# kyutai-labs/moshi

Hardware: AMD Instinct MI355X
Metric: 12.5 Hz frames/s end-to-end Mimi+Moshi-7B (higher is better)
Workload: dtype bf16

## Files before the change

### moshi_amd/csrc/mimi_engine.hip

```cpp
#include "mimi_kernels.h"
#include "mmi_graph.h"

#include <math.h>

namespace {

struct ConvW {
    float* wpk = nullptr;
    float* wpk_h = nullptr;
    float* bias = nullptr;
    int Cin = 0, Cout = 0, K = 1, S = 1, Mt = 0, Q = 0;
};

struct TrLayerW {
    ConvW in_proj, out_proj, lin1, lin2;
    float *n1w = nullptr, *n1b = nullptr, *n2w = nullptr, *n2b = nullptr, *ls1 = nullptr, *ls2 = nullptr;
    float *n1w_pk = nullptr, *n1b_pk = nullptr, *n2w_pk = nullptr, *n2b_pk = nullptr;
};

struct Buf {
    float* p = nullptr;
    int C = 0, ld = 0, H = 0;
    int lead = 0;
    float* pe = nullptr;
// ... 415 lines not shown
    }
    size_t n = (size_t)B * C * b->ld + b->lead;
    float* base = nullptr;
    MMI_HIP_CHECK(m->st.alloc(&base, n));
    MMI_HIP_CHECK(hipMemsetAsync(base, 0, n * sizeof(float), s));
    b->p = base + b->lead;
    return MMI_OK;
}

int alloc_twin(mmi_mimi* m, int B, Buf* b, hipStream_t s) {
    size_t n = (size_t)B * b->C * b->ld + b->lead;
    float* base = nullptr;
    MMI_HIP_CHECK(m->st.alloc(&base, n));
    MMI_HIP_CHECK(hipMemsetAsync(base, 0, n * sizeof(float), s));
    b->pe = base + b->lead;
    return MMI_OK;
}

HistDesc hist_of(const Buf& b, int T);
HistDesc hist_of_src(const Buf& b, int T) {
    Buf c = b;
    c.p = b.conv_src();
    return hist_of(c, T);
}

bool producer_packs(const mmi_mimi* m, int columns, const ConvW& w, int features) {
    return columns <= 128 && w.Q * 8 == features && !m->knobs.mimi_pack_launches;
}

int add_conv(mmi_mimi* m, MmiProgram& prog, ConvGemmArgs a, MmiArena* arena = nullptr) {
    ConvPlan p;
    int rc = plan_conv(m->knobs, arena ? *arena : m->st, a, &p);
    if (rc) return rc;
    prog.add([a, p](hipStream_t s) { return launch_conv_plan(s, a, p); });
    return MMI_OK;
}

int add_resblock(mmi_mimi* m, MmiProgram& prog, ConvGemmArgs a1, ConvGemmArgs a2, const ConvW& w2) {
    const int nblk = mmi_cdiv(a1.Ntot, 32);
    const long min_waves = m->knobs.res_fusion_min != MmiKnobs::UNSET ? m->knobs.res_fusion_min : 256;
    const bool fuse = a1.Ntot > 128 && a1.S == 1 && a2.K == 1 && a2.S == 1 && a1.Cout == a2.Cin && a1.Ntot == a2.Ntot &&
                      a1.T_out == a2.T_out && a1.Mt == 1 && w2.wpk_h && a2.Q <= 4 * a1.Mt &&
                      a2.Mt >= a1.Mt && (long)nblk * a1.Mt >= min_waves && !a1.first && !a2.first && !a1.res && !a1.scale && !a2.scale &&
                      a1.T_out % 32 == 0 && a1.Cin <= 64 * a1.Mt && a1.K <= 33 &&
                      a1.act_out == MMI_ACT_NONE && a2.act_out == MMI_ACT_NONE;
    if (!fuse) {
        int rc = add_conv(m, prog, a1);
        if (rc) return rc;
        return add_conv(m, prog, a2);
    }
    a2.wpk = w2.wpk_h;
    a2.elu_in = 0;
    ResBlockArgs ra;
    ra.a1 = a1; ra.a2 = a2;
    const int mt1 = a1.Mt;
    const size_t smem = ((size_t)((a1.Cin * (32 + a1.K - 1) + 3) & ~3) + (size_t)a1.Q * 8 + (mt1 > 1 ? (size_t)mt1 * 1024 : 0)) * sizeof(float);
    if (smem > 65536) return mmi_fail(MMI_ERR_UNSUPPORTED, "k_resblock: input window does not fit in LDS");
    prog.add([ra, nblk, smem](hipStream_t s) {
        MMI_LAUNCH((k_resblock<1, 4>), nblk, 64, smem, s, ra);
        MMI_CHECK_LAUNCH();
        return (int)MMI_OK;
    });
    return MMI_OK;
}

int add_quantize_ops(mmi_mimi* m, MmiProgram& prog, const float* latent, int lat_ld, int lat_off, int B, bool latent_packed = false) {
    const mmi_mimi_cfg& c = m->cfg;
    const int D = c.q_dimension, bins = c.q_bins;
    Buf in; in.p = const_cast<float*>(latent); in.C = c.dimension; in.ld = lat_ld; in.H = lat_off;
    Buf out; out.p = m->xq; out.C = 2 * D; out.ld = 1; out.H = 0;
    {
        ConvGemmArgs a = conv_args(m->q_in, in, lat_off, 1, out, 0, B, false);
        a.bp = m->qin_bp; a.partial = m->qin_part;
        a.x_packed = latent_packed ? 1 : 0;
        int rc = add_conv(m, prog, a);
        if (rc) return rc;
    }
    const int K = m->n_codebooks;
    const int nchunk = m->nchunk;
    const size_t smem = ((size_t)MMI_RVQ_CHUNK * (D + 4) + (size_t)8 * D) * sizeof(float);
    auto level = [&](int k, int slot) {
        const bool sem = k < c.q_n_q_semantic;
        RvqLevel L;
        L.x = m->xq + (sem ? 0 : D);
        L.E = m->E_all + (size_t)k * bins * D;
        L.e2 = m->e2_all + (size_t)k * bins;
        L.best_d = m->best_d + (size_t)slot * nchunk * m->max_batch;
        L.best_i = m->best_i + (size_t)slot * nchunk * m->max_batch;
        L.level = k;
        return L;
    };
    int* codes = m->codes_i32; const int nq = c.q_n_q;
    const bool pair = c.q_n_q_semantic == 1 && K >= 2 && !m->knobs.rvq_no_pair;
    for (int k = 0; k < K; ++k) {
        const RvqLevel a0 = level(k, 0);
        const bool two = pair && k == 0;
        const RvqLevel a1 = two ? level(1, 1) : a0;
        const int nz = two ? 2 : 1;
        prog.add([=](hipStream_t s) {
            MMI_LAUNCH(k_rvq_dist, dim3(nchunk, mmi_cdiv(B, 8), nz), 256, smem, s, a0, a1, 2 * D, B, D, bins);
            MMI_LAUNCH(k_rvq_select, dim3(B, nz), 256, 0, s, a0, a1, nchunk, 2 * D, codes, nq, B, D);
            MMI_CHECK_LAUNCH();
            return (int)MMI_OK;
        });
        if (two) ++k;
    }
    return MMI_OK;
}

int add_dequant_ops(mmi_mimi* m, MmiProgram& prog, int K, const Buf& out, int out_off, int B, bool k_from_device = false) {
    const mmi_mimi_cfg& c = m->cfg;
    const int D = c.q_dimension, bins = c.q_bins, nq = c.q_n_q, nsem = c.q_n_q_semantic;
    float* q2 = m->q2; const int* codes = m->dec_codes_i32; const float* E = m->E_all; const int* kdev = k_from_device ? m->dec_k_dev : nullptr;
    const bool packed = producer_packs(m, B, m->q_out, 2 * D);
    float* qp = packed ? m->qout_bp : nullptr; const int qQ = m->q_out.Q;
    prog.add([=](hipStream_t s) {
        MMI_LAUNCH(k_rvq_gather, mmi_cdiv(B * D, 256), 256, 0, s, codes, nq, K, E, bins, D, nsem, q2, B, kdev, qp, qQ);
        MMI_CHECK_LAUNCH();
        return (int)MMI_OK;
    });
    Buf in; in.p = m->q2; in.C = 2 * D; in.ld = 1; in.H = 0;
    ConvGemmArgs a = conv_args(m->q_out, in, 0, 1, out, out_off, B, false);
    a.bp = m->qout_bp; a.partial = m->qout_part;
    a.x_packed = packed ? 1 : 0;
    return add_conv(m, prog, a);
}

int add_transformer(mmi_mimi* m, MmiProgram& prog, const std::vector<TrLayerW>& layers, const Buf& xb, int off, int T,
                    float* kv, const long* offsets, int B, hipStream_t init_stream) {
    const mmi_mimi_cfg& c = m->cfg;
    const int d = c.tr_d_model, H = c.tr_num_heads, Dh = d / H, ff = c.tr_dim_feedforward, cap = c.tr_context;
    const int N = B * T;
    const bool packed = N <= 128;
    Buf y, qkv, att, hb;
    int rc;
    if ((rc = alloc_buf(m, B, d, 0, T, &y, init_stream))) return rc;
    if ((rc = alloc_buf(m, B, 3 * d, 0, T, &qkv, init_stream))) return rc;
    if ((rc = alloc_buf(m, B, d, 0, T, &att, init_stream))) return rc;
    if ((rc = alloc_buf(m, B, ff, 0, T, &hb, init_stream))) return rc;
    float *yp = nullptr, *attp = nullptr, *hbp = nullptr;
    const int nsub = mmi_cdiv(N, 32), Qd = mmi_cdiv(d, 8), Qff = mmi_cdiv(ff, 8);
    if (packed) {
        MMI_HIP_CHECK(m->st.alloc(&yp, (size_t)nsub * Qd * 256));
        MMI_HIP_CHECK(m->st.alloc(&attp, (size_t)nsub * Qd * 256));
        MMI_HIP_CHECK(m->st.alloc(&hbp, (size_t)nsub * Qff * 256));
        MMI_HIP_CHECK(hipMemsetAsync(yp, 0, (size_t)nsub * Qd * 256 * sizeof(float), init_stream));
        MMI_HIP_CHECK(hipMemsetAsync(attp, 0, (size_t)nsub * Qd * 256 * sizeof(float), init_stream));
        MMI_HIP_CHECK(hipMemsetAsync(hbp, 0, (size_t)nsub * Qff * 256 * sizeof(float), init_stream));
    }
    const size_t kv_layer = (size_t)B * H * cap * Dh;
    if (T > 2 || (Dh != 16 && Dh != 32 && Dh != 64))
        return mmi_fail(MMI_ERR_UNSUPPORTED, "Mimi attention: head dim 16/32/64 and 1 or 2 steps per frame are built");
    const size_t attn_smem = ((size_t)T * Dh + (((size_t)T * cap + 3) & ~(size_t)3) + (size_t)(256 / (Dh / 4)) * T * Dh + 8) * sizeof(float);
    auto add_norm = [&](const float* w, const float* bb) {
        const float* xp = xb.p; int xld = xb.ld; float* yn = y.p;
        prog.add([=](hipStream_t s) {
            MMI_LAUNCH(k_layernorm_ct, B * T, 64, 0, s, xp, xld, off, w, bb, yn, T, 0, d, T, 1e-5f, yp, Qd);
            MMI_CHECK_LAUNCH();
            return (int)MMI_OK;
        });
    };
    const bool fuse_ln = packed && d % 8 == 0 && Qd <= 64 && layers.size() > 0 && layers[0].n1w_pk;
    float* xrp = nullptr;
    if (fuse_ln) {
        MMI_HIP_CHECK(m->st.alloc(&xrp, (size_t)nsub * Qd * 256));
        MMI_HIP_CHECK(hipMemsetAsync(xrp, 0, (size_t)nsub * Qd * 256 * sizeof(float), init_stream));
    }
    bool x_is_packed = false;
    for (size_t l = 0; l < layers.size(); ++l) {
        const TrLayerW& L = layers[l];
        {
            ConvGemmArgs ai = conv_args(L.in_proj, y, 0, T, qkv, 0, B, false);
            if (fuse_ln && x_is_packed) {
                ai.x_packed = 1; ai.bp = xrp; ai.ln_w = L.n1w_pk; ai.ln_b = L.n1b_pk; ai.ln_eps = 1e-5f;
            } else {
                add_norm(L.n1w, L.n1b);
                if (packed) { ai.x_packed = 1; ai.bp = yp; }
            }
            if ((rc = add_conv(m, prog, ai))) return rc;
            MimiAttnArgs aa;
            aa.qkv = qkv.p; aa.kc = kv + (2 * l) * kv_layer; aa.vc = kv + (2 * l + 1) * kv_layer;
            aa.offsets = offsets; aa.out = att.p; aa.B = B; aa.H = H; aa.D = Dh; aa.T = T; aa.cap = cap;
            aa.context = c.tr_context; aa.max_period = c.tr_max_period;
            aa.outp = attp; aa.outQ = Qd;
            const bool one_pass = cap <= 16 * (256 / (Dh / 4)) && !m->knobs.mimi_attn_two_pass;
            prog.add([=](hipStream_t s) {
#define MMI_ATT(D_, T_) do { if (one_pass) MMI_LAUNCH((k_mimi_attn_1pass<D_, T_>), B * H, 256, 0, s, aa); \
                             else MMI_LAUNCH((k_mimi_attn<D_, T_>), B * H, 256, attn_smem, s, aa); } while (0)
                if (Dh == 64 && T == 2) MMI_ATT(64, 2);
                else if (Dh == 64 && T == 1) MMI_ATT(64, 1);
                else if (Dh == 32 && T == 2) MMI_ATT(32, 2);
                else if (Dh == 32 && T == 1) MMI_ATT(32, 1);
                else if (Dh == 16 && T == 2) MMI_ATT(16, 2);
                else if (Dh == 16 && T == 1) MMI_ATT(16, 1);
                else return mmi_fail(MMI_ERR_UNSUPPORTED, "Mimi attention: head dim 16/32/64 and 1 or 2 steps per frame are built");
#undef MMI_ATT
                MMI_CHECK_LAUNCH();
                return (int)MMI_OK;
            });
            ConvGemmArgs a = conv_args(L.out_proj, att, 0, T, xb, off, B, false);
            a.res = xb.p; a.res_ld = xb.ld; a.res_off = off; a.scale = L.ls1;
            if (packed) { a.x_packed = 1; a.bp = attp; }
            if (fuse_ln) { a.outp = xrp; a.outQ = Qd; x_is_packed = true; }
            if ((rc = add_conv(m, prog, a))) return rc;
        }
        {
            ConvGemmArgs a1 = conv_args(L.lin1, y, 0, T, hb, 0, B, false);
            a1.act_out = MMI_ACT_GELU;
            if (fuse_ln && x_is_packed) {
                a1.x_packed = 1; a1.bp = xrp; a1.ln_w = L.n2w_pk; a1.ln_b = L.n2b_pk; a1.ln_eps = 1e-5f;
                a1.out_mode = MMI_GOUT_PACKED; a1.outp = hbp; a1.outQ = Qff;
            } else {
                add_norm(L.n2w, L.n2b);
                if (packed) { a1.x_packed = 1; a1.bp = yp; a1.out_mode = MMI_GOUT_PACKED; a1.outp = hbp; a1.outQ = Qff; }
            }
            if ((rc = add_conv(m, prog, a1))) return rc;
            ConvGemmArgs a2 = conv_args(L.lin2, hb, 0, T, xb, off, B, false);
            a2.res = xb.p; a2.res_ld = xb.ld; a2.res_off = off; a2.scale = L.ls2;
            if (packed) { a2.x_packed = 1; a2.bp = hbp; }
            if (fuse_ln) { a2.outp = xrp; a2.outQ = Qd; x_is_packed = true; }
            if ((rc = add_conv(m, prog, a2))) return rc;
        }
    }
    return MMI_OK;
}

int upload_hist(mmi_mimi* m, std::vector<HistDesc>& h, int B, HistDesc** dev, int* n, int* rows, HistTable* tab = nullptr) {
    int acc = 0;
    std::vector<HistDesc> keep;
    for (auto& d : h) {
        if (d.H <= 0) continue;
        d.row_begin = acc;
        acc += B * d.C;
        keep.push_back(d);
    }
    *n = (int)keep.size();
    *rows = acc;
    if (tab) {
        memset(tab, 0, sizeof(*tab));
        tab->n = keep.size() <= MMI_HIST_MAX ? (int)keep.size() : -1;
        for (size_t i = 0; i < keep.size() && i < MMI_HIST_MAX; ++i) tab->d[i] = keep[i];
    }
    MMI_HIP_CHECK(m->st.alloc(dev, keep.size() ? keep.size() : 1));
    if (!keep.empty())
        MMI_HIP_CHECK(hipMemcpy(*dev, keep.data(), keep.size() * sizeof(HistDesc), hipMemcpyHostToDevice));
    return MMI_OK;
}

HistDesc hist_of(const Buf& b, int T) {
    HistDesc d;
    d.p = b.p; d.C = b.C; d.ld = b.ld; d.H = b.H; d.T = T; d.row_begin = 0;
    return d;
}

int add_commit(mmi_mimi* m, MmiProgram& prog, std::vector<HistDesc>& hist, int B, int T_tr, HistDesc** dev, int* n, int* n_rows, long* cnt,
               uint8_t* fi) {
    HistTable tab;
    int rc = upload_hist(m, hist, B, dev, n, n_rows, &tab);
    if (rc) return rc;
    HistDesc* hd = *dev; const int nh = *n, rows = *n_rows;
    const uint8_t* ex = m->exec;
    const bool one = tab.n >= 0 && !m->knobs.mimi_two_commits;
    prog.add([=](hipStream_t s) {
        if (one) {
            MMI_LAUNCH(k_commit_all, mmi_cdiv(rows + B, 256), 256, 0, s, tab, rows, ex, cnt, 1, T_tr, fi, B);
            MMI_CHECK_LAUNCH();
            return (int)MMI_OK;
        }
        if (rows > 0) MMI_LAUNCH(k_commit_history, mmi_cdiv(rows, 256), 256, 0, s, (const HistDesc*)hd, nh, rows, ex);
        MMI_LAUNCH(k_commit_counters, mmi_cdiv(B, 64), 64, 0, s, cnt, 1, T_tr, fi, ex, B);
        MMI_CHECK_LAUNCH();
        return (int)MMI_OK;
    });
    return MMI_OK;
}

int build_encoder(mmi_mimi* m, int B, hipStream_t s0) {
    const mmi_mimi_cfg& c = m->cfg;
    MmiProgram& prog = m->enc_prog;
    std::vector<HistDesc> hist;
    int rc;
    int T = c.frame_size;
    size_t ci = 0;
    if ((rc = alloc_buf(m, B, c.channels, c.kernel_size - 1, T, &m->enc_in, s0))) return rc;
    hist.push_back(hist_of(m->enc_in, T));
    Buf cur = m->enc_in;
    int mult = 1;
    {
        Buf nxt;
        if ((rc = alloc_buf(m, B, c.n_filters, c.residual_kernel_size - 1, T, &nxt, s0))) return rc;
        if ((rc = alloc_twin(m, B, &nxt, s0))) return rc;
        prog.site("enc.conv0");
        if ((rc = add_conv(m, prog, conv_args(m->enc_convs[ci++], cur, 0, T, nxt, nxt.H, B, false)))) return rc;
        hist.push_back(hist_of_src(nxt, T));
        cur = nxt;
    }
    for (int i = 0; i < c.n_ratios; ++i) {
        const int ratio = c.ratios[c.n_ratios - 1 - i];
        const int ch = mult * c.n_filters;
        Buf hid, nxt;
        if ((rc = alloc_buf(m, B, ch / c.compress, 0, T, &hid, s0))) return rc;
        if ((rc = alloc_buf(m, B, ch, ratio, T, &nxt, s0))) return rc;
        hid.elu = nxt.elu = true;
        prog.site("enc.res" + std::to_string(i));
        const ConvGemmArgs a1 = conv_args(m->enc_convs[ci++], cur, 0, T, hid, 0, B, true);
        const ConvW& w2 = m->enc_convs[ci++];
        ConvGemmArgs a = conv_args(w2, hid, 0, T, nxt, nxt.H, B, true);
        a.res = cur.p; a.res_ld = cur.ld; a.res_off = cur.H;
        if ((rc = add_resblock(m, prog, a1, a, w2))) return rc;
        hist.push_back(hist_of(nxt, T));
        cur = nxt;
        const int Tn = T / ratio;
        const int Hn = (i + 1 < c.n_ratios) ? c.residual_kernel_size - 1 : c.last_kernel_size - 1;
        Buf nx2;
        if ((rc = alloc_buf(m, B, 2 * ch, Hn, Tn, &nx2, s0))) return rc;
        if (i + 1 < c.n_ratios) { if ((rc = alloc_twin(m, B, &nx2, s0))) return rc; }
        else nx2.elu = true;
        prog.site("enc.down" + std::to_string(i));
        if ((rc = add_conv(m, prog, conv_args(m->enc_convs[ci++], cur, 0, Tn, nx2, nx2.H, B, true)))) return rc;
        hist.push_back(hist_of_src(nx2, Tn));
        cur = nx2;
        T = Tn;
        mult *= 2;
    }
    const int stride = c.resample_stride;
    Buf dsin;
    if ((rc = alloc_buf(m, B, c.dimension, 2 * stride - stride, T, &dsin, s0))) return rc;
    prog.site("enc.final");
    if ((rc = add_conv(m, prog, conv_args(m->enc_convs[ci++], cur, 0, T, dsin, dsin.H, B, true)))) return rc;
    hist.push_back(hist_of(dsin, T));
    {
        const int Dh = c.tr_d_model / c.tr_num_heads;
        size_t kvn = (size_t)2 * c.tr_num_layers * B * c.tr_num_heads * c.tr_context * Dh;
        MMI_HIP_CHECK(m->st.alloc(&m->enc_kv, kvn));
        MMI_HIP_CHECK(hipMemsetAsync(m->enc_kv, 0, kvn * sizeof(float), s0));
        prog.site("enc.tr");
        if ((rc = add_transformer(m, prog, m->enc_tr, dsin, dsin.H, T, m->enc_kv, m->counters, B, s0))) return rc;
    }
    const int T_tr = T;
    if (T % stride != 0 || T / stride != 1)
// ... 491 lines not shown
```

### moshi_amd/csrc/mimi_kernels.h

```cpp
#pragma once
#include "mmi_common.h"

__global__ void k_pack_a_f32(const float* __restrict__ W, float* __restrict__ P, int M, int Kd, long sm, long sk,
                             int Mt, int Q) {
    long idx = (long)blockIdx.x * blockDim.x + threadIdx.x;
    long total = (long)Mt * Q * 256;
    if (idx >= total) return;
    int e = (int)(idx & 3);
    int lane = (int)((idx >> 2) & 63);
    long rest = idx >> 8;
    int q = (int)(rest % Q);
    int mt = (int)(rest / Q);
    int m = mt * 32 + (lane & 31);
    int kd = (q * 4 + e) * 2 + (lane >> 5);
    float v = 0.f;
    if (m < M && kd < Kd) v = W[(long)m * sm + (long)kd * sk];
    P[idx] = v;
}

__global__ void k_copy2d_f32(const float* __restrict__ src, long sld, float* __restrict__ dst, long dld, int rows,
                             int cols) {
    long idx = (long)blockIdx.x * blockDim.x + threadIdx.x;
    if (idx >= (long)rows * cols) return;
    int r = (int)(idx / cols), c = (int)(idx % cols);
// ... 665 lines not shown
    float pv[8];
#pragma unroll
    for (int s = 0; s < 8; ++s) pv[s] = a.partial[((long)min(s, ksplit - 1) * a.Mt * 32 + co) * a.Npad + n];
    float x = 0.f;
#pragma unroll
    for (int s = 0; s < 8; ++s) x += s < ksplit ? pv[s] : 0.f;
    const int bq = mmi_fast_div(n, a.T_magic);
    int co1[1] = {co}, b1[1] = {bq}, t1[1] = {n - bq * a.T_out};
    bool ok1[1] = {true};
    float v1[1] = {x};
    mmi_conv_store_n<1>(a, co1, b1, t1, ok1, v1);
}

__global__ void k_convtr_combine(const float* __restrict__ tmp, const float* __restrict__ bias,
                                 float* __restrict__ partial, const uint8_t* __restrict__ exec, float* __restrict__ out,
                                 int out_ld, int out_off, int B, int Cout, int K, int S, int T_in, float* __restrict__ out2,
                                 int tmp_ld) {
    long idx = (long)blockIdx.x * blockDim.x + threadIdx.x;
    const int Tout = T_in * S;
    if (idx >= (long)B * Cout * Tout) return;
    int p = (int)(idx % Tout);
    long row = idx / Tout;
    int co = (int)(row % Cout);
    int b = (int)(row / Cout);
    int t = p / S, r = p - t * S;
    const float* trow = tmp + row * (long)K * tmp_ld;
    float v = trow[(long)r * tmp_ld + t];
    if (t > 0) v += trow[(long)(r + S) * tmp_ld + (t - 1)];
    if (bias) v += bias[co];
    if (t == 0) {
        long pi = row * (long)(K - S) + r;
        v += partial[pi];
        if (exec[b]) partial[pi] = trow[(long)(r + S) * tmp_ld + (T_in - 1)];
    }
    out[row * (long)out_ld + out_off + p] = v;
    if (out2) out2[row * (long)out_ld + out_off + p] = mmi_elu(v);
}

__global__ void k_upsample_dw(const float* __restrict__ x, int x_ld, int x_off, const float* __restrict__ w,
                              float* __restrict__ partial, const uint8_t* __restrict__ exec, float* __restrict__ out,
                              int out_ld, int out_off, int B, int C, int K, int S, int T_in) {
    long idx = (long)blockIdx.x * blockDim.x + threadIdx.x;
    const int Tout = T_in * S;
    if (idx >= (long)B * C * Tout) return;
    int p = (int)(idx % Tout);
    long row = idx / Tout;
    int c = (int)(row % C);
    int b = (int)(row / C);
    int t = p / S, r = p - t * S;
    const float* xr = x + row * (long)x_ld + x_off;
    float v = w[c * K + r] * xr[t];
    if (t > 0) v += w[c * K + r + S] * xr[t - 1];
    if (t == 0) {
        long pi = row * (long)(K - S) + r;
        v += partial[pi];
        if (exec[b]) partial[pi] = w[c * K + r + S] * xr[T_in - 1];
    }
    out[row * (long)out_ld + out_off + p] = v;
}

struct HistDesc {
    float* p;
    int C, ld, H, T;
    int row_begin;
};

__global__ void k_commit_history(const HistDesc* __restrict__ descs, int ndesc, int total_rows,
                                 const uint8_t* __restrict__ exec) {
    int gid = (int)(blockIdx.x * blockDim.x + threadIdx.x);
    if (gid >= total_rows) return;
    int d = 0;
    while (d + 1 < ndesc && descs[d + 1].row_begin <= gid) ++d;
    HistDesc h = descs[d];
    int row = gid - h.row_begin;
    int b = row / h.C;
    if (!exec[b]) return;
    float* r = h.p + (long)row * h.ld;
    for (int p = 0; p < h.H; ++p) r[p] = r[p + h.T];
}

#define MMI_HIST_MAX 16
struct HistTable {
    HistDesc d[MMI_HIST_MAX];
    int n;
};
__global__ void k_commit_all(HistTable tab, int total_rows, const uint8_t* __restrict__ exec, long* __restrict__ counters,
                             int n_counters, int inc, uint8_t* __restrict__ first, int B) {
    int gid = (int)(blockIdx.x * blockDim.x + threadIdx.x);
    if (gid >= total_rows) {
        gid -= total_rows;
        if (gid >= B || !exec[gid]) return;
        for (int i = 0; i < n_counters; ++i) counters[(long)i * B + gid] += inc;
        if (first) first[gid] = 0;
        return;
    }
    int d = 0;
#pragma unroll
    for (int i = 1; i < MMI_HIST_MAX; ++i)
        if (i < tab.n && tab.d[i].row_begin <= gid) d = i;
    const HistDesc h = tab.d[d];
    int row = gid - h.row_begin;
    int b = row / h.C;
    if (!exec[b]) return;
    float* r = h.p + (long)row * h.ld;
    for (int p = 0; p < h.H; ++p) r[p] = r[p + h.T];
}

__global__ void k_commit_counters(long* __restrict__ counters, int n_counters, int inc, uint8_t* __restrict__ first,
                                  const uint8_t* __restrict__ exec, int B) {
    int gid = (int)(blockIdx.x * blockDim.x + threadIdx.x);
    if (gid >= B) return;
    if (!exec[gid]) return;
    for (int i = 0; i < n_counters; ++i) counters[(long)i * B + gid] += inc;
    if (first) first[gid] = 0;
}

__global__ void k_reset_history(const HistDesc* __restrict__ descs, int ndesc, int total_rows,
                                const uint8_t* __restrict__ mask) {
    int gid = (int)(blockIdx.x * blockDim.x + threadIdx.x);
    if (gid >= total_rows) return;
    int d = 0;
    while (d + 1 < ndesc && descs[d + 1].row_begin <= gid) ++d;
    HistDesc h = descs[d];
    int row = gid - h.row_begin;
    int b = row / h.C;
    if (mask && !mask[b]) return;
    float* r = h.p + (long)row * h.ld;
    for (int p = 0; p < h.H; ++p) r[p] = 0.f;
}

__global__ void k_reset_rows_f32(float* __restrict__ buf, long n_per_row, int B, const uint8_t* __restrict__ mask) {
    long idx = (long)blockIdx.x * blockDim.x + threadIdx.x;
    if (idx >= (long)B * n_per_row) return;
    int b = (int)(idx / n_per_row);
    if (mask && !mask[b]) return;
    buf[idx] = 0.f;
}

__global__ void k_reset_counters(long* __restrict__ counters, int n_counters, uint8_t* __restrict__ first,
                                 uint8_t* __restrict__ exec, int B, const uint8_t* __restrict__ mask) {
    int gid = (int)(blockIdx.x * blockDim.x + threadIdx.x);
    if (gid >= B) return;
    if (mask && !mask[gid]) return;
    for (int i = 0; i < n_counters; ++i) counters[(long)i * B + gid] = 0;
    if (first) first[gid] = 1;
    exec[gid] = 1;
}

__global__ void k_set_mask(uint8_t* __restrict__ dst, const uint8_t* __restrict__ src, int B) {
    int gid = (int)(blockIdx.x * blockDim.x + threadIdx.x);
    if (gid < B) dst[gid] = src[gid] ? 1 : 0;
}

__global__ __launch_bounds__(64) void k_layernorm_ct(const float* __restrict__ x, int x_ld, int x_off,
                                                     const float* __restrict__ w, const float* __restrict__ bvec,
                                                     float* __restrict__ y, int y_ld, int y_off, int C, int T,
                                                     float eps, float* __restrict__ yp, int yQ) {
    const int b = blockIdx.x / T, t = blockIdx.x % T;
    const int lane = threadIdx.x;
    const float* xc = x + (long)b * C * x_ld + x_off + t;
    constexpr int NR = 16;
    float xv[NR], wv[NR], bv[NR];
    float s = 0.f;
#pragma unroll
    for (int i = 0; i < NR; ++i) {
        const int c = lane + i * 64;
        const int cc = c < C ? c : 0;
        xv[i] = xc[(long)cc * x_ld];
        wv[i] = w[cc];
        bv[i] = bvec[cc];
    }
#pragma unroll
    for (int i = 0; i < NR; ++i) s += (lane + i * 64) < C ? xv[i] : 0.f;
#pragma unroll
    for (int m = 32; m >= 1; m >>= 1) s += mmi_shfl_xor(s, m);
    const float mean = s / (float)C;
    float v = 0.f;
#pragma unroll
    for (int i = 0; i < NR; ++i) {
        const float d = xv[i] - mean;
        v += (lane + i * 64) < C ? d * d : 0.f;
    }
#pragma unroll
    for (int m = 32; m >= 1; m >>= 1) v += mmi_shfl_xor(v, m);
    const float rstd = mmi_rsqrtf(v / (float)C + eps);
    float* yc = y + (long)b * C * y_ld + y_off + t;
#pragma unroll
    for (int i = 0; i < NR; ++i) {
        const int c = lane + i * 64;
        if (c < C) {
            const float o = (xv[i] - mean) * rstd * wv[i] + bv[i];
            if (yp) yp[mmi_bp_index(c, blockIdx.x, yQ)] = o;
            else yc[(long)c * y_ld] = o;
        }
    }
}

struct MimiAttnArgs {
    const float* qkv;
    float* kc;
    float* vc;
    const long* offsets;
    float* out;
    float* outp;
    int outQ;
    int B, H, D, T, cap, context;
    float max_period;
};

template <int D, int T>
__global__ __launch_bounds__(256) void k_mimi_attn(MimiAttnArgs a) {
    constexpr int LPR = D / 4;
    constexpr int RPB = 256 / LPR;
    const int b = blockIdx.x / a.H, h = blockIdx.x % a.H;
    const int tid = threadIdx.x, lane = tid & 63, wave = tid >> 6;
    const int cap = a.cap;
    MMI_DYN_SHARED(float, sm);
    float* qs = sm;
    float* sc = qs + T * D;
    float* red = sc + ((T * cap + 3) & ~3);
    const long off = a.offsets[b];
    const int HD = a.H * D;
    const float* qrow = a.qkv + (long)b * 3 * HD * T;
    float* kcb = a.kc + ((long)b * a.H + h) * cap * D;
    float* vcb = a.vc + ((long)b * a.H + h) * cap * D;

    for (int i = tid; i < T * (D / 2); i += 256) {
        const int t = i / (D / 2), j = i % (D / 2);
        const float freq = expf((float)j * (-logf(a.max_period) * 2.0f / (float)D));
        const float ts = (float)(off + t);
        const float ang = freq * ts;
        const float c = cosf(ang), s = sinf(ang);
        const float qr = qrow[(long)(h * D + 2 * j) * T + t], qi = qrow[(long)(h * D + 2 * j + 1) * T + t];
        const float kr = qrow[(long)(HD + h * D + 2 * j) * T + t], ki = qrow[(long)(HD + h * D + 2 * j + 1) * T + t];
        float q_re, q_im, k_re, k_im;
        mmi_rope_rotate(qr, qi, c, s, q_re, q_im);
        mmi_rope_rotate(kr, ki, c, s, k_re, k_im);
        qs[t * D + 2 * j] = q_re;
        qs[t * D + 2 * j + 1] = q_im;
        const int slot = (int)((off + t) % cap);
        kcb[(long)slot * D + 2 * j] = k_re;
        kcb[(long)slot * D + 2 * j + 1] = k_im;
    }
    for (int i = tid; i < T * D; i += 256) {
        const int t = i / D, d = i % D;
        const int slot = (int)((off + t) % cap);
        vcb[(long)slot * D + d] = qrow[(long)(2 * HD + h * D + d) * T + t];
    }
    __syncthreads();

    const long last = off + T - 1;
    const int end_index = (int)(last % cap);
    const long end_new = off + T;
    const int L = (int)(end_new < (long)cap ? end_new : (long)cap);
    const float scale = 1.0f / sqrtf((float)D);
    const int seg = tid % LPR, rsub = tid / LPR;
    f32x4 qv[T];
#pragma unroll
    for (int t = 0; t < T; ++t) qv[t] = *reinterpret_cast<const f32x4*>(qs + t * D + seg * 4);
    constexpr int NP = 8;
    for (int s0 = 0; s0 < L; s0 += NP * RPB) {
        f32x4 kk[NP];
#pragma unroll
        for (int i = 0; i < NP; ++i) kk[i] = *reinterpret_cast<const f32x4*>(kcb + (long)min(s0 + i * RPB + rsub, L - 1) * D + seg * 4);
#pragma unroll
        for (int i = 0; i < NP; ++i) {
            const int slot = s0 + i * RPB + rsub;
            const int delta = slot - end_index;
            const long pos = delta <= 0 ? last + delta : last + delta - cap;
#pragma unroll
            for (int t = 0; t < T; ++t) {
                float dv = (qv[t][0] * kk[i][0] + qv[t][1] * kk[i][1]) + (qv[t][2] * kk[i][2] + qv[t][3] * kk[i][3]);
#pragma unroll
                for (int m = LPR / 2; m >= 1; m >>= 1) dv += mmi_shfl_xor(dv, m);
                if (seg == 0 && slot < L) {
                    const long dq = (off + t) - pos;
                    const bool ok = pos >= 0 && dq >= 0 && dq < a.context;
                    sc[t * cap + slot] = ok ? dv * scale : -INFINITY;
                }
            }
        }
    }
    __syncthreads();

    if (wave < T) {
        const int t = wave;
        float m = -INFINITY;
        for (int slot = lane; slot < L; slot += 64) m = fmaxf(m, sc[t * cap + slot]);
#pragma unroll
        for (int x = 32; x >= 1; x >>= 1) m = fmaxf(m, mmi_shfl_xor(m, x));
        float sum = 0.f;
        for (int slot = lane; slot < L; slot += 64) {
            const float e = expf(sc[t * cap + slot] - m);
            sc[t * cap + slot] = e;
            sum += e;
        }
#pragma unroll
        for (int x = 32; x >= 1; x >>= 1) sum += mmi_shfl_xor(sum, x);
        const float inv = 1.0f / sum;
        for (int slot = lane; slot < L; slot += 64) sc[t * cap + slot] *= inv;
    }
    __syncthreads();

    float acc[T][4];
#pragma unroll
    for (int t = 0; t < T; ++t)
#pragma unroll
        for (int e = 0; e < 4; ++e) acc[t][e] = 0.f;
    for (int s0 = 0; s0 < L; s0 += NP * RPB) {
        f32x4 vv[NP];
#pragma unroll
        for (int i = 0; i < NP; ++i) vv[i] = *reinterpret_cast<const f32x4*>(vcb + (long)min(s0 + i * RPB + rsub, L - 1) * D + seg * 4);
#pragma unroll
        for (int i = 0; i < NP; ++i) {
            const int slot = s0 + i * RPB + rsub;
#pragma unroll
            for (int t = 0; t < T; ++t) {
                const float pr = slot < L ? sc[t * cap + slot] : 0.f;
#pragma unroll
                for (int e = 0; e < 4; ++e) acc[t][e] += pr * vv[i][e];
            }
        }
    }
#pragma unroll
    for (int t = 0; t < T; ++t)
        *reinterpret_cast<f32x4*>(red + (rsub * T + t) * D + seg * 4) = f32x4{acc[t][0], acc[t][1], acc[t][2], acc[t][3]};
    __syncthreads();
    for (int i = tid; i < T * D; i += 256) {
        const int t = i / D, d = i % D;
        float s = 0.f;
#pragma unroll 8
        for (int r = 0; r < RPB; ++r) s += red[(r * T + t) * D + d];
        if (a.outp) a.outp[mmi_bp_index(h * D + d, b * T + t, a.outQ)] = s;
        else a.out[((long)b * HD + h * D + d) * T + t] = s;
    }
}

template <int D, int T>
__global__ __launch_bounds__(256) void k_mimi_attn_1pass(MimiAttnArgs a) {
    constexpr int LPR = D / 4;
    constexpr int RPB = 256 / LPR;
    constexpr int IT = 16;
    const int b = blockIdx.x / a.H, h = blockIdx.x % a.H;
    const int tid = threadIdx.x, lane = tid & 63, wave = tid >> 6;
    const int cap = a.cap;
    MMI_SHARED __attribute__((aligned(16))) float qs[T * D];
    MMI_SHARED __attribute__((aligned(16))) float kn[T * D];
    MMI_SHARED __attribute__((aligned(16))) float vn[T * D];
    MMI_SHARED __attribute__((aligned(16))) float red[4 * T * D];
    MMI_SHARED float mw[4 * T];
    MMI_SHARED float sw[4 * T];
    const long off = a.offsets[b];
    const int HD = a.H * D;
    const float* qrow = a.qkv + (long)b * 3 * HD * T;
    float* kcb = a.kc + ((long)b * a.H + h) * cap * D;
    float* vcb = a.vc + ((long)b * a.H + h) * cap * D;
    const long last = off + T - 1;
    const int end_index = (int)(last % cap);
    const long end_new = off + T;
    const int L = (int)(end_new < (long)cap ? end_new : (long)cap);
    const int seg = tid % LPR, rsub = tid / LPR;

    f32x4 kk[IT], vv[IT];
#pragma unroll
    for (int i = 0; i < IT; ++i) {
        const long r = (long)min(i * RPB + rsub, L - 1) * D + seg * 4;
        kk[i] = *reinterpret_cast<const f32x4*>(kcb + r);
        vv[i] = *reinterpret_cast<const f32x4*>(vcb + r);
    }

    for (int i = tid; i < T * (D / 2); i += 256) {
        const int t = i / (D / 2), j = i % (D / 2);
        const float freq = expf((float)j * (-logf(a.max_period) * 2.0f / (float)D));
        const float ang = freq * (float)(off + t);
        const float c = cosf(ang), s = sinf(ang);
        const float qr = qrow[(long)(h * D + 2 * j) * T + t], qi = qrow[(long)(h * D + 2 * j + 1) * T + t];
        const float kr = qrow[(long)(HD + h * D + 2 * j) * T + t], ki = qrow[(long)(HD + h * D + 2 * j + 1) * T + t];
        mmi_rope_rotate(qr, qi, c, s, qs[t * D + 2 * j], qs[t * D + 2 * j + 1]);
        mmi_rope_rotate(kr, ki, c, s, kn[t * D + 2 * j], kn[t * D + 2 * j + 1]);
    }
    for (int i = tid; i < T * D; i += 256) {
        const int t = i / D, d = i % D;
        vn[i] = qrow[(long)(2 * HD + h * D + d) * T + t];
    }
    __syncthreads();
    for (int i = tid; i < T * D; i += 256) {
        const int t = i / D, d = i % D;
        const long slot = (off + t) % cap;
        kcb[slot * D + d] = kn[i];
        vcb[slot * D + d] = vn[i];
    }

    const float scale = 1.0f / sqrtf((float)D);
    f32x4 qv[T];
    int newslot[T];
#pragma unroll
    for (int t = 0; t < T; ++t) {
        qv[t] = *reinterpret_cast<const f32x4*>(qs + t * D + seg * 4);
        newslot[t] = (int)((off + t) % cap);
    }
    float sc[T][IT];
    float mx[T];
#pragma unroll
    for (int t = 0; t < T; ++t) mx[t] = -INFINITY;
#pragma unroll
    for (int i = 0; i < IT; ++i) {
        const int slot = i * RPB + rsub;
#pragma unroll
        for (int t = 0; t < T; ++t)
            if (slot == newslot[t]) {
                kk[i] = *reinterpret_cast<const f32x4*>(kn + t * D + seg * 4);
                vv[i] = *reinterpret_cast<const f32x4*>(vn + t * D + seg * 4);
            }
        const int delta = slot - end_index;
        const long pos = delta <= 0 ? last + delta : last + delta - cap;
#pragma unroll
        for (int t = 0; t < T; ++t) {
            float dv = (qv[t][0] * kk[i][0] + qv[t][1] * kk[i][1]) + (qv[t][2] * kk[i][2] + qv[t][3] * kk[i][3]);
#pragma unroll
            for (int m = LPR / 2; m >= 1; m >>= 1) dv += mmi_shfl_xor(dv, m);
            const long dq = (off + t) - pos;
            const bool ok = slot < L && pos >= 0 && dq >= 0 && dq < a.context;
            sc[t][i] = ok ? dv * scale : -INFINITY;
            mx[t] = fmaxf(mx[t], sc[t][i]);
        }
    }
    float acc[T][4], sum[T];
#pragma unroll
    for (int t = 0; t < T; ++t) {
#pragma unroll
        for (int m = LPR; m < 64; m <<= 1) mx[t] = fmaxf(mx[t], mmi_shfl_xor(mx[t], m));
        const float mref = mx[t] == -INFINITY ? 0.f : mx[t];
        sum[t] = 0.f;
#pragma unroll
        for (int e = 0; e < 4; ++e) acc[t][e] = 0.f;
#pragma unroll
        for (int i = 0; i < IT; ++i) {
            const float p = expf(sc[t][i] - mref);
            sum[t] += p;
#pragma unroll
            for (int e = 0; e < 4; ++e) acc[t][e] += p * vv[i][e];
        }
#pragma unroll
        for (int m = LPR; m < 64; m <<= 1) {
            sum[t] += mmi_shfl_xor(sum[t], m);
#pragma unroll
            for (int e = 0; e < 4; ++e) acc[t][e] += mmi_shfl_xor(acc[t][e], m);
        }
        if (lane < LPR) {
            *reinterpret_cast<f32x4*>(red + (wave * T + t) * D + seg * 4) = f32x4{acc[t][0], acc[t][1], acc[t][2], acc[t][3]};
            if (lane == 0) { mw[wave * T + t] = mx[t]; sw[wave * T + t] = sum[t]; }
        }
    }
    __syncthreads();
    for (int i = tid; i < T * D; i += 256) {
        const int t = i / D, d = i % D;
        float m = mw[t];
#pragma unroll
        for (int w = 1; w < 4; ++w) m = fmaxf(m, mw[w * T + t]);
        float num = 0.f, den = 0.f;
#pragma unroll
        for (int w = 0; w < 4; ++w) {
            const float f = expf(mw[w * T + t] - m);
            num += f * red[(w * T + t) * D + d];
            den += f * sw[w * T + t];
        }
        const float o = num / den;
        if (a.outp) a.outp[mmi_bp_index(h * D + d, b * T + t, a.outQ)] = o;
        else a.out[((long)b * HD + h * D + d) * T + t] = o;
    }
}

#define MMI_RVQ_CHUNK 32
struct RvqLevel {
    float* x;
    const float* E;
    const double* e2;
    double* best_d;
    int* best_i;
    int level;
};

__global__ __launch_bounds__(256) void k_rvq_dist(RvqLevel l0, RvqLevel l1, int x_rstride, int Bn, int D, int bins) {
    const RvqLevel& L = blockIdx.z == 0 ? l0 : l1;
    const float* __restrict__ x = L.x;
    const float* __restrict__ E = L.E;
    const double* __restrict__ e2 = L.e2;
    double* __restrict__ best_d = L.best_d;
    int* __restrict__ best_i = L.best_i;
    MMI_DYN_SHARED(float, sm);
    const int ldE = D + 4;
    float* Es = sm;
    float* xs = sm + MMI_RVQ_CHUNK * ldE;
    const int chunk = blockIdx.x;
    const int c0 = chunk * MMI_RVQ_CHUNK;
    const int tid = threadIdx.x;
    const int rg0 = (int)blockIdx.y * 8;
    const int D4 = D >> 2;
    {
        const int r = tid >> 3, j0 = tid & 7;
        const int code = min(c0 + r, bins - 1);
        for (int j = j0; j < D4; j += 8)
            *reinterpret_cast<f32x4*>(Es + r * ldE + 4 * j) = *reinterpret_cast<const f32x4*>(E + (long)code * D + 4 * j);
        if (r < 8) {
            const int row = min(rg0 + r, Bn - 1);
            for (int j = j0; j < D4; j += 8)
                *reinterpret_cast<f32x4*>(xs + r * D + 4 * j) = *reinterpret_cast<const f32x4*>(x + (long)row * x_rstride + 4 * j);
        }
    }
    __syncthreads();
    const int c = tid & 31, g = tid >> 5;
    const bool cvalid = (c0 + c) < bins;
    const double en = cvalid ? e2[c0 + c] : 0.0;
    const int r = rg0 + g;
    const bool rvalid = r < Bn;
    double a0 = 0.0, a1 = 0.0, a2 = 0.0, a3 = 0.0;
    for (int j = 0; j < D4; ++j) {
        const f32x4 ev = *reinterpret_cast<const f32x4*>(Es + c * ldE + 4 * j);
        const f32x4 xv = *reinterpret_cast<const f32x4*>(xs + g * D + 4 * j);
        a0 += (double)ev[0] * (double)xv[0];
        a1 += (double)ev[1] * (double)xv[1];
        a2 += (double)ev[2] * (double)xv[2];
        a3 += (double)ev[3] * (double)xv[3];
    }
    const double acc = (a0 + a1) + (a2 + a3);
    double dist = (cvalid && rvalid) ? en - 2.0 * acc : INFINITY;
    int idx = c0 + c;
#pragma unroll
    for (int m = 16; m >= 1; m >>= 1) {
        double od = mmi_shfl_xor(dist, m);
        int oi = mmi_shfl_xor(idx, m);
        if (od < dist || (od == dist && oi < idx)) { dist = od; idx = oi; }
    }
    if (c == 0 && rvalid) { best_d[(long)chunk * Bn + r] = dist; best_i[(long)chunk * Bn + r] = idx; }
}

__global__ __launch_bounds__(256) void k_rvq_select(RvqLevel l0, RvqLevel l1, int nchunk, int x_rstride, int* __restrict__ codes,
                                                    int codes_rstride, int Bn, int D) {
    const RvqLevel& L = blockIdx.y == 0 ? l0 : l1;
    const double* __restrict__ best_d = L.best_d;
    const int* __restrict__ best_i = L.best_i;
    float* __restrict__ x = L.x;
    const float* __restrict__ E = L.E;
    const int level = L.level;
    const int r = blockIdx.x;
    MMI_SHARED int widx;
    if (threadIdx.x < 64) {
        double bd = INFINITY;
        int bi = 0x7fffffff;
        for (int ch = threadIdx.x; ch < nchunk; ch += 64) {
            double d = best_d[(long)ch * Bn + r];
            int i = best_i[(long)ch * Bn + r];
            if (d < bd || (d == bd && i < bi)) { bd = d; bi = i; }
        }
#pragma unroll
        for (int m = 32; m >= 1; m >>= 1) {
            double od = mmi_shfl_xor(bd, m);
            int oi = mmi_shfl_xor(bi, m);
            if (od < bd || (od == bd && oi < bi)) { bd = od; bi = oi; }
        }
// ... 47 lines not shown
```

### moshi_amd/csrc/mmi_knobs.h

```cpp
#pragma once
#include <limits.h>
#include <stdio.h>
#include <stdlib.h>
#include <atomic>
#include <string>
#include <vector>

struct MmiKnobs {
    static constexpr int UNSET = INT_MIN;

    bool no_graph = false;
    char debug_poison = 0;
    std::vector<std::string> skip_sites;

    int lm_tile = 0;
    int dep_tile = 0;
    bool no_dep_in_group = false;
    int gemm_ksplit = 0;
    bool gemm_osplit_set = false;
    int gemm_osplit = UNSET;
    bool gemm_osplit_all = false;
    char gemm_lds = 0;
    int gemm_lds_grid = UNSET;
    char gemm_once = 0;
    bool no_norm_fusion = false;
    bool q8_act_bf16 = false;
    bool q8_u2 = false;
    bool q8_tiles_serial = false;
    bool rows_groups = false;
    int rows_ntw = 0;
    bool attn_split = false;
    int attn_ns = 0;
    int attn_solo = UNSET;
    bool attn_merge_kernel = false;
    bool no_dep_attn_fusion = false;
    bool dep_attn0_launch = false;
    bool no_precapture = false;
    bool debug_trace = false;
    std::string debug_trace_prefix;
    std::string debug_dump;

    int conv_mtb = 0;
    int conv_w = 0;
    int conv_ksplit = 0;
    long res_fusion_min = UNSET;
    bool mimi_no_align = false;
    bool rvq_no_pair = false;
    bool mimi_pack_launches = false;
    bool mimi_attn_two_pass = false;
    bool mimi_two_commits = false;

    int duplex_codec_cus = 0;
    char duplex_prio = 0;
};

inline void mmi_knob_warn_once(std::atomic<bool>& said, const char* name, const char* value, const char* what) {
    if (!said.exchange(true)) fprintf(stderr, "moshi_mi: %s=%s is set: %s\n", name, value, what);
}

inline MmiKnobs mmi_knobs_from_env() {
    MmiKnobs k;
    auto present = [](const char* name) { return getenv(name) != nullptr; };
    auto first = [](const char* name) { const char* e = getenv(name); return e ? e[0] : (char)0; };
    auto number = [](const char* name, int absent) { const char* e = getenv(name); return e ? atoi(e) : absent; };
    auto one_of = [](int v, std::initializer_list<int> ok) { for (int o : ok) if (v == o) return v; return 0; };

    {
        const char* e = getenv("MMI_NO_GRAPH");
        k.no_graph = e && e[0] && e[0] != '0';
    }
    {
        const char p = first("MMI_DEBUG_POISON");
        k.debug_poison = p == '1' || p == '0' ? p : (char)0;
    }
    if (const char* e = getenv("MMI_SKIP_SITES")) {
        const std::string all(e);
        for (size_t i = 0; i <= all.size();) {
            const size_t j = all.find(',', i);
            const std::string pre = all.substr(i, j == std::string::npos ? std::string::npos : j - i);
            if (!pre.empty()) k.skip_sites.push_back(pre);
            if (j == std::string::npos) break;
            i = j + 1;
        }
        static std::atomic<bool> said{false};
        if (!k.skip_sites.empty()) mmi_knob_warn_once(said, "MMI_SKIP_SITES", e, "launch-list sites are left out, the outputs are garbage (timing experiments only)");
    }

    k.lm_tile = one_of(number("MMI_LM_TILE", 0), {16, 32});
    k.dep_tile = number("MMI_DEP_TILE", 0);
    k.no_dep_in_group = present("MMI_NO_DEP_IN_GROUP");
    {
        const int v = number("MMI_GEMM_KSPLIT", 0);
        k.gemm_ksplit = v >= 1 && v <= 4 ? v : 0;
    }
    if (const char* e = getenv("MMI_GEMM_OSPLIT")) {
        k.gemm_osplit_set = true;
        if (e[0]) { k.gemm_osplit = atoi(e); k.gemm_osplit_all = e[1] == 'a'; }
    }
    k.gemm_lds = first("MMI_GEMM_LDS");
    k.gemm_lds_grid = number("MMI_GEMM_LDS_GRID", MmiKnobs::UNSET);
    k.gemm_once = first("MMI_GEMM_ONCE");
    k.no_norm_fusion = present("MMI_NO_NORM_FUSION");
    k.q8_act_bf16 = first("MMI_Q8_ACT") == 'b';
    k.q8_u2 = first("MMI_Q8_U") == '2';
    k.q8_tiles_serial = first("MMI_Q8_TILES") == 's';
    {
        const char* e = getenv("MMI_ROWS_GROUPS");
        k.rows_groups = e && e[0] && e[0] != '0';
    }
    k.rows_ntw = one_of(number("MMI_ROWS_NTW", 0), {1, 2});
    k.attn_split = first("MMI_ATTN") == 's';
    {
        const int v = number("MMI_ATTN_NS", 0);
        k.attn_ns = v >= 1 && v <= 16 ? v : 0;
    }
    k.attn_solo = number("MMI_ATTN_SOLO", MmiKnobs::UNSET);
    k.attn_merge_kernel = first("MMI_ATTN_MERGE") == 'k';
    k.no_dep_attn_fusion = present("MMI_NO_DEP_ATTN_FUSION");
    k.dep_attn0_launch = present("MMI_DEP_ATTN0_LAUNCH");
    k.no_precapture = present("MMI_NO_PRECAPTURE");
    if (const char* e = getenv("MMI_DEBUG_TRACE")) { k.debug_trace = true; k.debug_trace_prefix = e; }
    if (const char* e = getenv("MMI_DEBUG_DUMP")) k.debug_dump = e;

    k.conv_mtb = one_of(number("MMI_CONV_MTB", 0), {1, 2, 4});
    k.conv_w = one_of(number("MMI_CONV_W", 0), {1, 2, 4, 8});
    {
        const int v = number("MMI_CONV_KSPLIT", 0);
        k.conv_ksplit = v >= 1 && v <= 8 ? v : 0;
    }
    if (const char* e = getenv("MMI_MIMI_RES_FUSION_MIN")) k.res_fusion_min = atol(e);
    k.mimi_no_align = present("MMI_MIMI_NO_ALIGN");
    k.rvq_no_pair = present("MMI_RVQ_NO_PAIR");
    k.mimi_pack_launches = present("MMI_MIMI_PACK_LAUNCHES");
    k.mimi_attn_two_pass = present("MMI_MIMI_ATTN_TWO_PASS");
    k.mimi_two_commits = present("MMI_MIMI_TWO_COMMITS");

    if (const char* e = getenv("MMI_DUPLEX_CODEC_CUS")) {
        const int v = atoi(e);
        static std::atomic<bool> said{false};
        if (v > 0 && v < 256) {
            k.duplex_codec_cus = v;
            mmi_knob_warn_once(said, "MMI_DUPLEX_CODEC_CUS", e, "the duplex pipeline's codec streams run on a CU mask (experiment)");
        } else if (e[0]) mmi_knob_warn_once(said, "MMI_DUPLEX_CODEC_CUS", e, "ignored, the CU count must be 1..255");
    }
    if (const char* e = getenv("MMI_DUPLEX_PRIO")) {
        static std::atomic<bool> said{false};
        if (e[0] == 'c' || e[0] == 'n') {
            k.duplex_prio = e[0];
            mmi_knob_warn_once(said, "MMI_DUPLEX_PRIO", e, "the duplex pipeline's stream priorities are not the shipped ones (A/B)");
        } else if (e[0]) mmi_knob_warn_once(said, "MMI_DUPLEX_PRIO", e, "ignored, the values are codec / none");
    }
    return k;
}
```

Baseline: 4480.

## Precompute Mimi RoPE table in layernorm launch and prefetch KV before offset load

Extra blocks are added to the first layernorm launch of each transformer so they compute the cos/sin RoPE table once per frame. The one-pass attention kernel then reads this table instead of evaluating expf/cosf/sinf in every layer and head. The kernel also issues its first K/V cache loads before reading the offset, clamping them to the cache capacity, and zeroes V for slots past the valid length. The aim is to cut transcendental work and hide load latency, at the cost of a small buffer and extra blocks in the layernorm launch.

```diff
diff --git a/moshi_amd/csrc/mimi_engine.hip b/moshi_amd/csrc/mimi_engine.hip
--- a/moshi_amd/csrc/mimi_engine.hip
+++ b/moshi_amd/csrc/mimi_engine.hip
@@ -591,10 +591,21 @@
     if (T > 2 || (Dh != 16 && Dh != 32 && Dh != 64))
         return mmi_fail(MMI_ERR_UNSUPPORTED, "Mimi attention: head dim 16/32/64 and 1 or 2 steps per frame are built");
     const size_t attn_smem = ((size_t)T * Dh + (((size_t)T * cap + 3) & ~(size_t)3) + (size_t)(256 / (Dh / 4)) * T * Dh + 8) * sizeof(float);
+    const bool one_pass = cap <= 16 * (256 / (Dh / 4)) && !m->knobs.mimi_attn_two_pass;
+    float* rope = nullptr;
+    if (one_pass && !m->knobs.mimi_rope_in_kernel && !layers.empty()) {
+        MMI_HIP_CHECK(m->st.alloc(&rope, (size_t)N * Dh));
+        MMI_HIP_CHECK(hipMemsetAsync(rope, 0, (size_t)N * Dh * sizeof(float), init_stream));
+    }
+    bool rope_filled = false;
+    const float max_period = c.tr_max_period;
     auto add_norm = [&](const float* w, const float* bb) {
         const float* xp = xb.p; int xld = xb.ld; float* yn = y.p;
+        float* rp = rope_filled ? nullptr : rope;
+        rope_filled = true;
         prog.add([=](hipStream_t s) {
-            MMI_LAUNCH(k_layernorm_ct, B * T, 64, 0, s, xp, xld, off, w, bb, yn, T, 0, d, T, 1e-5f, yp, Qd);
+            MMI_LAUNCH(k_layernorm_ct, rp ? 2 * B * T : B * T, 64, 0, s, xp, xld, off, w, bb, yn, T, 0, d, T, 1e-5f, yp, Qd, B * T, rp, offsets, Dh,
+                       max_period);
             MMI_CHECK_LAUNCH();
             return (int)MMI_OK;
         });
@@ -621,10 +632,10 @@
             aa.qkv = qkv.p; aa.kc = kv + (2 * l) * kv_layer; aa.vc = kv + (2 * l + 1) * kv_layer;
             aa.offsets = offsets; aa.out = att.p; aa.B = B; aa.H = H; aa.D = Dh; aa.T = T; aa.cap = cap;
             aa.context = c.tr_context; aa.max_period = c.tr_max_period;
-            aa.outp = attp; aa.outQ = Qd;
-            const bool one_pass = cap <= 16 * (256 / (Dh / 4)) && !m->knobs.mimi_attn_two_pass;
+            aa.outp = attp; aa.outQ = Qd; aa.rope = rope;
             prog.add([=](hipStream_t s) {
-#define MMI_ATT(D_, T_) do { if (one_pass) MMI_LAUNCH((k_mimi_attn_1pass<D_, T_>), B * H, 256, 0, s, aa); \
+#define MMI_ATT(D_, T_) do { if (one_pass && rope) MMI_LAUNCH((k_mimi_attn_1pass<D_, T_, true>), B * H, 256, 0, s, aa); \
+                             else if (one_pass) MMI_LAUNCH((k_mimi_attn_1pass<D_, T_, false>), B * H, 256, 0, s, aa); \
                              else MMI_LAUNCH((k_mimi_attn<D_, T_>), B * H, 256, attn_smem, s, aa); } while (0)
                 if (Dh == 64 && T == 2) MMI_ATT(64, 2);
                 else if (Dh == 64 && T == 1) MMI_ATT(64, 1);
diff --git a/moshi_amd/csrc/mimi_kernels.h b/moshi_amd/csrc/mimi_kernels.h
--- a/moshi_amd/csrc/mimi_kernels.h
+++ b/moshi_amd/csrc/mimi_kernels.h
@@ -841,12 +841,31 @@
     if (gid < B) dst[gid] = src[gid] ? 1 : 0;
 }
 
+__device__ __forceinline__ void mmi_mimi_rope_cs(float max_period, int D, long pos, int j, float& c, float& sn) {
+    const float freq = expf((float)j * (-logf(max_period) * 2.0f / (float)D));
+    const float ang = freq * (float)pos;
+    c = cosf(ang);
+    sn = sinf(ang);
+}
+
 __global__ __launch_bounds__(64) void k_layernorm_ct(const float* __restrict__ x, int x_ld, int x_off,
                                                      const float* __restrict__ w, const float* __restrict__ bvec,
                                                      float* __restrict__ y, int y_ld, int y_off, int C, int T,
-                                                     float eps, float* __restrict__ yp, int yQ) {
+                                                     float eps, float* __restrict__ yp, int yQ,
+                                                     int n_norm, float* __restrict__ rope, const long* __restrict__ offsets, int Dh,
+                                                     float max_period) {
+    const int lane = threadIdx.x;
+    if (blockIdx.x >= n_norm) {
+        const int bt = (int)blockIdx.x - n_norm;
+        const long pos = offsets[bt / T] + bt % T;
+        if (lane < Dh / 2) {
+            float c, sn;
+            mmi_mimi_rope_cs(max_period, Dh, pos, lane, c, sn);
+            *reinterpret_cast<f32x2*>(rope + ((long)bt * (Dh / 2) + lane) * 2) = f32x2{c, sn};
+        }
+        return;
+    }
     const int b = blockIdx.x / T, t = blockIdx.x % T;
-    const int lane = threadIdx.x;
     const float* xc = x + (long)b * C * x_ld + x_off + t;
     constexpr int NR = 16;
     float xv[NR], wv[NR], bv[NR];
@@ -895,6 +914,7 @@
     int outQ;
     int B, H, D, T, cap, context;
     float max_period;
+    const float* rope;
 };
 
 template <int D, int T>
@@ -916,10 +936,8 @@
 
     for (int i = tid; i < T * (D / 2); i += 256) {
         const int t = i / (D / 2), j = i % (D / 2);
-        const float freq = expf((float)j * (-logf(a.max_period) * 2.0f / (float)D));
-        const float ts = (float)(off + t);
-        const float ang = freq * ts;
-        const float c = cosf(ang), s = sinf(ang);
+        float c, s;
+        mmi_mimi_rope_cs(a.max_period, D, off + t, j, c, s);
         const float qr = qrow[(long)(h * D + 2 * j) * T + t], qi = qrow[(long)(h * D + 2 * j + 1) * T + t];
         const float kr = qrow[(long)(HD + h * D + 2 * j) * T + t], ki = qrow[(long)(HD + h * D + 2 * j + 1) * T + t];
         float q_re, q_im, k_re, k_im;
@@ -1025,11 +1043,12 @@
     }
 }
 
-template <int D, int T>
+template <int D, int T, bool TAB>
 __global__ __launch_bounds__(256) void k_mimi_attn_1pass(MimiAttnArgs a) {
     constexpr int LPR = D / 4;
     constexpr int RPB = 256 / LPR;
     constexpr int IT = 16;
+    constexpr int NE = RPB >= 64 ? 1 : 64 / RPB;
     const int b = blockIdx.x / a.H, h = blockIdx.x % a.H;
     const int tid = threadIdx.x, lane = tid & 63, wave = tid >> 6;
     const int cap = a.cap;
@@ -1039,30 +1058,37 @@
     MMI_SHARED __attribute__((aligned(16))) float red[4 * T * D];
     MMI_SHARED float mw[4 * T];
     MMI_SHARED float sw[4 * T];
-    const long off = a.offsets[b];
     const int HD = a.H * D;
     const float* qrow = a.qkv + (long)b * 3 * HD * T;
     float* kcb = a.kc + ((long)b * a.H + h) * cap * D;
     float* vcb = a.vc + ((long)b * a.H + h) * cap * D;
+    const int seg = tid % LPR, rsub = tid / LPR;
+
+    f32x4 kk[IT], vv[IT];
+    auto request = [&](int i, int last_slot) {
+        const unsigned r = (unsigned)min(i * RPB + rsub, last_slot) * (unsigned)(D * 4) + (unsigned)(seg * 16);
+        kk[i] = *reinterpret_cast<const f32x4*>(reinterpret_cast<const uint8_t*>(kcb) + r);
+        vv[i] = *reinterpret_cast<const f32x4*>(reinterpret_cast<const uint8_t*>(vcb) + r);
+    };
+#pragma unroll
+    for (int i = 0; i < NE; ++i) request(i, cap - 1);
+    const long off = a.offsets[b];
     const long last = off + T - 1;
     const int end_index = (int)(last % cap);
     const long end_new = off + T;
     const int L = (int)(end_new < (long)cap ? end_new : (long)cap);
-    const int seg = tid % LPR, rsub = tid / LPR;
-
-    f32x4 kk[IT], vv[IT];
-#pragma unroll
-    for (int i = 0; i < IT; ++i) {
-        const long r = (long)min(i * RPB + rsub, L - 1) * D + seg * 4;
-        kk[i] = *reinterpret_cast<const f32x4*>(kcb + r);
-        vv[i] = *reinterpret_cast<const f32x4*>(vcb + r);
-    }
+#pragma unroll
+    for (int i = NE; i < IT; ++i) request(i, L - 1);
 
     for (int i = tid; i < T * (D / 2); i += 256) {
         const int t = i / (D / 2), j = i % (D / 2);
-        const float freq = expf((float)j * (-logf(a.max_period) * 2.0f / (float)D));
-        const float ang = freq * (float)(off + t);
-        const float c = cosf(ang), s = sinf(ang);
+        float c, s;
+        if constexpr (TAB) {
+            const f32x2 cs = *reinterpret_cast<const f32x2*>(a.rope + ((long)(b * T + t) * (D / 2) + j) * 2);
+            c = cs[0]; s = cs[1];
+        } else {
+            mmi_mimi_rope_cs(a.max_period, D, off + t, j, c, s);
+        }
         const float qr = qrow[(long)(h * D + 2 * j) * T + t], qi = qrow[(long)(h * D + 2 * j + 1) * T + t];
         const float kr = qrow[(long)(HD + h * D + 2 * j) * T + t], ki = qrow[(long)(HD + h * D + 2 * j + 1) * T + t];
         mmi_rope_rotate(qr, qi, c, s, qs[t * D + 2 * j], qs[t * D + 2 * j + 1]);
@@ -1095,6 +1121,7 @@
 #pragma unroll
     for (int i = 0; i < IT; ++i) {
         const int slot = i * RPB + rsub;
+        if (slot >= L) vv[i] = f32x4{0.f, 0.f, 0.f, 0.f};
 #pragma unroll
         for (int t = 0; t < T; ++t)
             if (slot == newslot[t]) {
diff --git a/moshi_amd/csrc/mmi_knobs.h b/moshi_amd/csrc/mmi_knobs.h
--- a/moshi_amd/csrc/mmi_knobs.h
+++ b/moshi_amd/csrc/mmi_knobs.h
@@ -48,6 +48,7 @@
     bool rvq_no_pair = false;
     bool mimi_pack_launches = false;
     bool mimi_attn_two_pass = false;
+    bool mimi_rope_in_kernel = false;
     bool mimi_two_commits = false;
 
     int duplex_codec_cus = 0;
@@ -133,6 +134,7 @@
     k.rvq_no_pair = present("MMI_RVQ_NO_PAIR");
     k.mimi_pack_launches = present("MMI_MIMI_PACK_LAUNCHES");
     k.mimi_attn_two_pass = present("MMI_MIMI_ATTN_TWO_PASS");
+    k.mimi_rope_in_kernel = first("MMI_MIMI_ROPE") == 'k';
     k.mimi_two_commits = present("MMI_MIMI_TWO_COMMITS");
 
     if (const char* e = getenv("MMI_DUPLEX_CODEC_CUS")) {
```

Measured after the change: 4464. About the same (-0.4%).
